# alexrenz/AdaPM

Measured on AMD Instinct MI355X. Metric: pull_push_ops_per_s, higher is better.
Workload: dtype fp32; 1 GPU; model=kge_complex_dim512, entities=10000000, relations=1000, dim=512, neg_samples=16, global_batch=16384, triples=90000000, parallelism=ps-async-dp1, fused_step=True, warmup_extra_steps=400

## Files before the change

adapm_amd/csrc/core.cpp:

```cpp
#include <torch/extension.h>
#include <ATen/Parallel.h>

#include <algorithm>
#include <atomic>
#include <condition_variable>
#include <cstring>
#include <limits>
#include <deque>
#include <map>
#include <queue>
#include <tuple>
#include <memory>
#include <mutex>
#include <random>
#include <thread>
#include <chrono>
#include <unordered_map>
#include <unordered_set>
#include <cstdio>
#include <vector>

#include "common.h"
#include "kernels.h"
#include "ops.h"
// ... 229 lines not shown
    adopt(current_stream(dev_));
    state_.copy_(h);
  }

  std::vector<uint64_t> export_state() {
    torch::Tensor h;
    {
      std::lock_guard<std::mutex> g(mu_);
      adopt(current_stream(dev_));
      h = state_.slice(0, 0, USTREAM_GEN_WORDS).cpu();
    }
    const uint64_t* p = reinterpret_cast<const uint64_t*>(h.data_ptr<int64_t>());
    return std::vector<uint64_t>(p, p + USTREAM_GEN_WORDS);
  }

  torch::Tensor draw(int64_t n, int64_t slack = -1) {
    TORCH_CHECK(n >= 0, "UniformStream.draw: n must be >= 0");
    auto opt = torch::TensorOptions().dtype(torch::kInt64).device(dev_);
    auto out = torch::empty({n}, opt);
    if (n == 0) return out;
    if (slack < 0) {
      double p = (double)thr_ / 4294967296.0;
      double w0 = (double)n / (1.0 - p);
      slack = (int64_t)std::ceil(w0 - (double)n + 8.0 * std::sqrt(w0 * p) / (1.0 - p)) + 16;
    }
    const int64_t words = n + slack;
    std::lock_guard<std::mutex> g(mu_);
    void* st = current_stream(dev_);
    adopt(st);
    auto tmp = torch::empty({ustream_tmp_words(words)}, opt);
    uint64_t* sp = reinterpret_cast<uint64_t*>(state_.data_ptr<int64_t>());
    if (dev_.is_cuda()) {
#ifdef ADAPM_WITH_HIP
      uniform_draw_gpu(sp, lo_, excl_, thr_, n, words, out.data_ptr<int64_t>(),
                       tmp.data_ptr<int64_t>(), st);
#else
      TORCH_CHECK(false, "UniformStream: built without HIP");
#endif
    } else {
      uniform_draw_cpu(sp, lo_, excl_, thr_, n, words, out.data_ptr<int64_t>(),
                       tmp.data_ptr<int64_t>());
    }
    return out;
  }

  int64_t lo() const { return lo_; }
  int64_t hi() const { return hi_; }
  const torch::Device& device() const { return dev_; }

 private:
// ... 2223 lines not shown
      const int64_t n = t->numel();
      for (int64_t i = 0; i < n; ++i) {
        int64_t k = kp[i];
        dst[i] = k;
        bad |= ((uint64_t)k >= lim);
      }
      dst += n;
    }
    if (bad)
      for (auto* t : parts) check_key_range(*t);
    hk.blob = blob;
    return hk;
  }

  StagedKeys upload_keys(const char* name, const HostKeys& hk, uint32_t* tags = nullptr,
                         const int64_t* dev_keys = nullptr, int64_t n_dev = 0) {
    const torch::Tensor& blob = hk.blob;
    const int64_t total = blob.numel();
    StagedKeys sk;
    sk.dev = torch::empty({total}, torch::TensorOptions().dtype(torch::kInt64).device(dev_));
#ifdef ADAPM_WITH_HIP
    auto stream = c10::hip::getCurrentHIPStreamMasqueradingAsCUDA(dev_.index());
    const bool ok =
        tags ? keys_land_gpu(tags, sk.dev.data_ptr<int64_t>(), blob.data_ptr<int64_t>(), total,
                             dev_keys, n_dev, (void*)stream.stream())
             : copy_keys_gpu(sk.dev.data_ptr<int64_t>(), blob.data_ptr<int64_t>(), total,
                             (void*)stream.stream());
    TORCH_CHECK(ok, name, ": the pinned key staging buffer is not visible to the device");
    at::getHostAllocator(at::kCUDA)->record_event(
        blob.data_ptr(), blob.storage().data_ptr().get_context(), stream.unwrap());
#else
    TORCH_CHECK(false, name, ": built without HIP");
#endif
    const int64_t* dp = sk.dev.data_ptr<int64_t>();
    for (int64_t n : hk.n) {
      sk.ptr.push_back(dp);
      dp += n;
    }
    return sk;
  }

  std::tuple<torch::Tensor, torch::Tensor> kge_step_fused_impl(
      const torch::Tensor& keys_s, const torch::Tensor& keys_r, const torch::Tensor& keys_o,
// ... 4 lines not shown
    int64_t B = keys_s.numel();
    TORCH_CHECK(keys_r.numel() == B && keys_o.numel() == B);
    TORCH_CHECK(N >= 0 && (3 + N) * B < (int64_t)ROWTAG_SHARED,
                "kge_step_fused: too many keys in one step");
    HostKeys hk;
    StagedKeys sk;
    torch::Tensor drawn;
    const int64_t* kn = nullptr;
    if (us) {
      TORCH_CHECK(us->lo() >= 0 && us->hi() <= num_keys_, "kge_step_fused_sampled: stream range [",
                  us->lo(), ", ", us->hi(), ") exceeds the store's ", num_keys_, " keys");
      TORCH_CHECK(us->device() == dev_,
                  "kge_step_fused_sampled: stream is not on the store's device");
      TORCH_CHECK(N >= 0 && B * N > 0, "kge_step_fused_sampled: nothing to draw");
      hk = host_keys({&keys_s, &keys_r, &keys_o});
      drawn = us->draw(B * N);
      kn = drawn.data_ptr<int64_t>();
    } else {
      TORCH_CHECK(keys_neg->numel() == B * N);
      hk = host_keys({&keys_s, &keys_r, &keys_o, keys_neg});
    }
    const int64_t n_dev = us ? B * N : 0;

    auto loss = torch::empty({B}, torch::TensorOptions().dtype(torch::kFloat32).device(dev_));
    void* st = current_stream(dev_);
    {
      InflightGuard g(this);
      std::unique_lock<std::mutex> mg(fused_mu_);
      if (fused_plain_ok(st)) {
        auto* tags = reinterpret_cast<uint32_t*>(fused_tags_.data_ptr<int32_t>());
        uint32_t* bits = tags + 32 * rowtag_words(num_keys_);
        sk = upload_keys("kge_step_fused", hk, tags, kn, n_dev);
        if (!us) kn = sk.ptr[3];
        RowTagKeys tk{{sk.ptr[0], kn, nullptr, nullptr}, {hk.blob.numel(), n_dev, 0, 0}, 2};
        rowtag_flag_gpu(tags, tk, st);
        rowtag_bits_gpu(tags, bits, tk, st);
        kge_complex_step_fused_gpu(
            slab_.data, sk.ptr[0], sk.ptr[1], sk.ptr[2], kn, loss.data_ptr<float>(), (int)B,
            (int)N, (int)D, Slab::padded(uniform_len_), world_, (float)lr, (float)eps, st, bits,
            fused_shared_stat_.defined()
                ? reinterpret_cast<unsigned long long*>(fused_shared_stat_.data_ptr<int64_t>())
                : nullptr);
        stat_fused_plain_ += 1;
      } else {
        mg.unlock();
        sk = upload_keys("kge_step_fused", hk);
        if (!us) kn = sk.ptr[3];
        kge_complex_step_fused_gpu(slab_.data, sk.ptr[0], sk.ptr[1], sk.ptr[2], kn,
                                   loss.data_ptr<float>(), (int)B, (int)N, (int)D,
                                   Slab::padded(uniform_len_), world_, (float)lr, (float)eps, st);
        stat_fused_atomic_ += 1;
      }
    }
    count_fused_ops(3 * B + B * N);
    return {loss, drawn};
  }

  torch::Tensor kge_step_fused(torch::Tensor keys_s, torch::Tensor keys_r, torch::Tensor keys_o,
                               torch::Tensor keys_neg, int64_t N, int64_t D, double lr,
                               double eps) {
// ... 44 lines not shown
    const int64_t n_dev = us ? B * (N + NS) : 0;

    auto loss = torch::empty({B}, torch::TensorOptions().dtype(torch::kFloat32).device(dev_));
    void* st = current_stream(dev_);
    {
      InflightGuard g(this);
      std::unique_lock<std::mutex> mg(fused_mu_);
      const bool plain = fused_plain_ok(st);
      uint32_t *tags = nullptr, *bits = nullptr;
      if (plain) {
        tags = reinterpret_cast<uint32_t*>(fused_tags_.data_ptr<int32_t>());
        bits = tags + 32 * rowtag_words(num_keys_);
      } else {
        mg.unlock();
      }
      sk = upload_keys(name, hk, tags, kno, n_dev);
      if (!us) kno = sk.ptr[3], kns = sk.ptr[4];
      if (plain) {
        RowTagKeys tk{{sk.ptr[0], kno, nullptr, nullptr}, {hk.blob.numel(), n_dev, 0, 0}, 2};
        rowtag_flag_gpu(tags, tk, st);
        rowtag_bits_gpu(tags, bits, tk, st);
      }
      kge_complex_step_sides_fused_gpu(
          slab_.data, sk.ptr[0], sk.ptr[1], sk.ptr[2], kno, kns, loss.data_ptr<float>(), (int)B,
          (int)N, (int)NS, (int)D, Slab::padded(uniform_len_), world_, (float)lr, (float)eps,
          (float)gamma_e, (float)gamma_r, st, bits,
          plain && fused_shared_stat_.defined()
              ? reinterpret_cast<unsigned long long*>(fused_shared_stat_.data_ptr<int64_t>())
              : nullptr);
      (plain ? stat_fused_plain_ : stat_fused_atomic_) += 1;
    }
    count_fused_ops(3 * B + B * (N + NS));
    return {loss, drawn};
  }

  torch::Tensor kge_step_sides_fused(torch::Tensor keys_s, torch::Tensor keys_r,
                                     torch::Tensor keys_o, torch::Tensor keys_neg_o,
                                     torch::Tensor keys_neg_s, int64_t N, int64_t NS, int64_t D,
                                     double lr, double eps, double gamma_e, double gamma_r) {
    return std::get<0>(kge_step_sides_fused_impl(keys_s, keys_r, keys_o, &keys_neg_o,
                                                 &keys_neg_s, nullptr, N, NS, D, lr, eps,
                                                 gamma_e, gamma_r));
  }

// ... 1126 lines not shown
    total += n;
  }
  TORCH_CHECK(total < (int64_t)ROWTAG_SHARED, "rowtag_shared_mask: too many occurrences");
  const int64_t words = rowtag_words(num_keys);
  auto tags = torch::empty({33 * words}, torch::TensorOptions().dtype(torch::kInt32).device(dev));
  auto* tp = reinterpret_cast<uint32_t*>(tags.data_ptr<int32_t>());
  void* st = current_stream(dev);
  rowtag_tag_gpu(tp, tk, st);
  rowtag_flag_gpu(tp, tk, st);
  rowtag_bits_gpu(tp, tp + 32 * words, tk, st);
  auto all = torch::cat(dk);
  auto word = tags.narrow(0, 32 * words, words).index_select(0, all.div(32, "floor"));
  return word.bitwise_right_shift(all.remainder(32).to(torch::kInt32)).bitwise_and(1).eq(1);
}

}

PYBIND11_MODULE(TORCH_EXTENSION_NAME, m) {
  using namespace adapm;
  m.def("hip_available", &hip_available);
  m.def("kge_complex_step", &kge_complex_step, py::call_guard<py::gil_scoped_release>());
  m.def("kge_complex_step_sides", &kge_complex_step_sides,
        py::call_guard<py::gil_scoped_release>());
  m.def("alias_draw", &alias_draw, py::call_guard<py::gil_scoped_release>());
  m.def("rescal_step", &rescal_step, py::call_guard<py::gil_scoped_release>());
  m.def("rescal_step_grouped", &rescal_step_grouped, py::call_guard<py::gil_scoped_release>());
  m.def("kge_complex_score", &kge_complex_score, py::call_guard<py::gil_scoped_release>());
  m.def("rank_count", &rank_count, py::arg("q"), py::arg("cand"), py::arg("base"),
        py::arg("counts"), py::arg("K"), py::arg("max_blocks") = 0,
        py::call_guard<py::gil_scoped_release>());
  m.def("pair_scores", &pair_scores, py::arg("q"), py::arg("cand"), py::arg("owner"),
        py::arg("out"), py::arg("K"), py::call_guard<py::gil_scoped_release>());
  m.def("w2v_sgns_step", &w2v_sgns_step, py::call_guard<py::gil_scoped_release>());
  m.def("mf_update_step", &mf_update_step, py::call_guard<py::gil_scoped_release>());
  m.def("mf_loss", &mf_loss, py::call_guard<py::gil_scoped_release>());
  m.def("slab_op", &slab_op, py::arg("op"), py::arg("dev"), py::arg("host"), py::arg("src_off"),
        py::arg("dst_off"), py::arg("lens"), py::arg("aux_off"), py::arg("buf"), py::arg("set"),
        py::call_guard<py::gil_scoped_release>());
  m.def("slab_keys_op", &slab_keys_op, py::arg("op"), py::arg("dev"), py::arg("keys"),
        py::arg("len"), py::arg("plen"), py::arg("world"), py::arg("rank"), py::arg("buf"),
        py::arg("set"), py::call_guard<py::gil_scoped_release>());
  m.def("rowtag_shared_mask", &rowtag_shared_mask, py::arg("keys"), py::arg("num_keys"),
        py::call_guard<py::gil_scoped_release>());
  py::class_<UniformStream>(m, "UniformStream")
      .def(py::init<int64_t, int64_t, std::string>(), py::arg("lo"), py::arg("hi"),
           py::arg("device"))
      .def_static("supported", &UniformStream::supported)
      .def("import_state", &UniformStream::import_state, py::call_guard<py::gil_scoped_release>())
      .def("export_state", &UniformStream::export_state, py::call_guard<py::gil_scoped_release>())
      .def("draw", &UniformStream::draw, py::arg("n"), py::arg("slack") = -1,
           py::call_guard<py::gil_scoped_release>())
      .def("lo", &UniformStream::lo)
      .def("hi", &UniformStream::hi);
  py::class_<Server>(m, "Server")
      .def(py::init<int64_t, torch::Tensor, int, int, int, int, std::string, double, int, bool,
                    int64_t, int64_t, double>(),
           py::arg("num_keys"), py::arg("value_lengths"), py::arg("rank"), py::arg("world"),
           py::arg("num_channels"), py::arg("num_workers"), py::arg("device"),
           py::arg("capacity_factor") = 2.0, py::arg("techniques") = 0,
           py::arg("location_caches") = true, py::arg("device_cap_floats") = 0,
           py::arg("host_spill_floats") = 0, py::arg("sync_threshold") = 0.0)
      .def("pull", &Server::pull, py::call_guard<py::gil_scoped_release>())
      .def("push", &Server::push, py::call_guard<py::gil_scoped_release>())
      .def("pull_if_local", &Server::pull_if_local, py::call_guard<py::gil_scoped_release>())
      .def("is_local", &Server::is_local)
      .def("intent", &Server::intent, py::call_guard<py::gil_scoped_release>())
      .def("advance_clock", &Server::advance_clock)
      .def("current_clock", &Server::current_clock)
// ... 57 lines not shown
```

adapm_amd/csrc/kernels.h:

```cpp
#pragma once
#include <cstdint>

namespace adapm {

constexpr int STEP_MAX_LANES = 8 * 256;

void kge_complex_step_gpu(const float* s, const float* r, const float* o, const float* neg,
                          float* ds, float* dr, float* do_, float* dneg, float* loss,
                          int B, int N, int D, float lr, float eps, void* stream);
void kge_complex_step_cpu(const float* s, const float* r, const float* o, const float* neg,
                          float* ds, float* dr, float* do_, float* dneg, float* loss,
                          int B, int N, int D, float lr, float eps);

void kge_complex_step_sides_gpu(const float* s, const float* r, const float* o,
                                const float* neg_o, const float* neg_s, float* ds, float* dr,
                                float* do_, float* dneg_o, float* dneg_s, float* loss, int B,
                                int N, int NS, int D, float lr, float eps, float gamma_e,
                                float gamma_r, void* stream);
void kge_complex_step_sides_cpu(const float* s, const float* r, const float* o,
                                const float* neg_o, const float* neg_s, float* ds, float* dr,
                                float* do_, float* dneg_o, float* dneg_s, float* loss, int B,
                                int N, int NS, int D, float lr, float eps, float gamma_e,
                                float gamma_r);

constexpr uint32_t ROWTAG_SHARED = 0xFFFFFFFFu;
struct RowTagKeys {
  const int64_t* keys[4];
  int64_t n[4];
  int count;
};
inline int64_t rowtag_words(int64_t rows) { return (rows + 31) / 32; }
void rowtag_tag_gpu(uint32_t* tags, const RowTagKeys& ks, void* stream);
void rowtag_flag_gpu(uint32_t* tags, const RowTagKeys& ks, void* stream);
void rowtag_bits_gpu(const uint32_t* tags, uint32_t* bits, const RowTagKeys& ks, void* stream);

bool keys_land_gpu(uint32_t* tags, int64_t* dst, const int64_t* src_host, int64_t n_copy,
                   const int64_t* dev_keys, int64_t n_dev, void* stream);

void kge_complex_step_fused_gpu(float* slab, const int64_t* keys_s, const int64_t* keys_r,
                                const int64_t* keys_o, const int64_t* keys_neg, float* loss,
                                int B, int N, int D, int32_t plen, int world, float lr,
                                float eps, void* stream, const uint32_t* bits = nullptr,
                                unsigned long long* shared_stat = nullptr);

void kge_complex_step_sides_fused_gpu(float* slab, const int64_t* keys_s, const int64_t* keys_r,
                                      const int64_t* keys_o, const int64_t* keys_neg_o,
                                      const int64_t* keys_neg_s, float* loss, int B, int N,
                                      int NS, int D, int32_t plen, int world, float lr,
                                      float eps, float gamma_e, float gamma_r, void* stream,
                                      const uint32_t* bits = nullptr,
                                      unsigned long long* shared_stat = nullptr);
void kge_complex_step_sides_fused_offs_cpu(float* slab, const int64_t* offs_s,
                                           const int64_t* offs_r, const int64_t* offs_o,
                                           const int64_t* offs_neg_o, const int64_t* offs_neg_s,
                                           float* loss, int B, int N, int NS, int D, float lr,
                                           float eps, float gamma_e, float gamma_r);

void kge_complex_step_fused_offs_cpu(float* slab, const int64_t* offs_s, const int64_t* offs_r,
                                     const int64_t* offs_o, const int64_t* offs_neg, float* loss,
                                     int B, int N, int D, float lr, float eps);
void w2v_sgns_step_fused_offs_cpu(float* slab, const int64_t* offs_ctr, const int64_t* offs_ctx,
                                  const int64_t* offs_neg, float* loss, int B, int N, int D,
                                  float lr, float eps);
void mf_update_step_fused_offs_cpu(float* slab, const int64_t* offs_w, const int64_t* offs_h,
                                   const float* x, float* loss, int B, int R, float lr,
                                   float lambda, float eps);
// ... 29 lines not shown
                        float* loss, int B, int R, float lr, float lambda, float eps,
                        void* stream);
void mf_update_step_cpu(const float* w, const float* h, const float* x, float* dw, float* dh,
                        float* loss, int B, int R, float lr, float lambda, float eps);

void mf_loss_gpu(const float* w, const float* h, const float* x, double* acc2, int B, int R,
                 float lambda, void* stream);
void mf_loss_cpu(const float* w, const float* h, const float* x, float* out2, int B, int R,
                 float lambda);

void alias_draw_gpu(const float* prob, const int32_t* alias, int64_t n, uint64_t seed,
                    int64_t N, int64_t* out, void* stream);
void alias_draw_cpu(const float* prob, const int32_t* alias, int64_t n, uint64_t seed,
                    int64_t N, int64_t* out);

void uniform_draw_gpu(uint64_t* state, int64_t lo, uint32_t excl, uint32_t thr, int64_t n,
                      int64_t words, int64_t* out, int64_t* tmp, void* stream);
void uniform_draw_cpu(uint64_t* state, int64_t lo, uint32_t excl, uint32_t thr, int64_t n,
                      int64_t words, int64_t* out, int64_t* tmp);

bool copy_keys_gpu(int64_t* dst, const int64_t* src_host, int64_t n, void* stream);

}

namespace adapm {


void kge_complex_score_mfma_gpu(const float* s, const float* r, const float* cand,
                                float* scores, float* qbuf, int B, int E, int D, void* stream);

void rank_count_gpu(const float* Q, const float* C, const float* base, int32_t* counts, int B,
                    int E, int K, int qstride, int cstride, int max_blocks, void* stream);
// ... 22 lines not shown
```

adapm_amd/csrc/kernels_hip.hip:

```cpp
#include <hip/hip_runtime.h>
#include <algorithm>
#include <type_traits>

#include "kernels.h"
#include "ustream.h"

namespace adapm {

#define KT 256

static inline unsigned grid_for(int64_t n, int64_t cap = 16384) {
  return (unsigned)std::min(std::max<int64_t>(n, 1), cap);
}

static_assert(STEP_MAX_LANES == 8 * KT, "dispatch_kpt stops at KPT = 8");
template <typename F>
static inline void dispatch_kpt(int lanes, F&& f) {
  if (lanes <= KT) f(std::integral_constant<int, 1>{});
  else if (lanes <= 2 * KT) f(std::integral_constant<int, 2>{});
  else if (lanes <= 4 * KT) f(std::integral_constant<int, 4>{});
  else f(std::integral_constant<int, 8>{});
}

__device__ inline float block_reduce_sum(float v, float* lds) {
// ... 462 lines not shown
}

namespace adapm {
void alias_draw_gpu(const float* prob, const int32_t* alias, int64_t n, uint64_t seed,
                    int64_t N, int64_t* out, void* stream) {
  if (N == 0) return;
  hipLaunchKernelGGL(k_alias_draw, dim3(grid_for((N + 255) / 256, 4096)), dim3(256), 0,
                     (hipStream_t)stream, prob, alias, n, seed, N, out);
}
}

namespace adapm {

static_assert(USTREAM_BLOCK == KT, "one chunk per thread of a KT workgroup");

__device__ inline int64_t block_reduce_i64(int64_t v, int64_t* lds) {
  for (int off = 32; off > 0; off >>= 1) v += __shfl_xor(v, off, 64);
  if ((threadIdx.x & 63) == 0) lds[threadIdx.x >> 6] = v;
  __syncthreads();
  int64_t out = 0;
  for (int i = 0; i < KT / 64; ++i) out += lds[i];
  __syncthreads();
  return out;
}

template <typename T>
__device__ inline T* ustream_block_keys(T* tmp, int64_t nb, int64_t block) {
  return tmp + USTREAM_TMP_COUNTS + nb + block * (KT * USTREAM_CHUNK) + threadIdx.x;
}

__global__ void __launch_bounds__(KT)
k_ustream_gen(const uint64_t* __restrict__ state, UStreamRange r, int64_t words, int64_t chunks,
              int64_t* __restrict__ tmp, int64_t nb) {
  __shared__ int64_t lds[KT / 64];
  const int64_t c = (int64_t)blockIdx.x * KT + threadIdx.x;
  int64_t cnt = 0;
  if (c < chunks)
    cnt = ustream_gen_chunk(state, r, words, c, ustream_block_keys(tmp, nb, blockIdx.x), KT);
  cnt = block_reduce_i64(cnt, lds);
  if (threadIdx.x == 0) {
    tmp[USTREAM_TMP_COUNTS + blockIdx.x] = cnt;
  }
}

__global__ void __launch_bounds__(KT)
k_ustream_compact(uint64_t* __restrict__ state, UStreamRange r, int64_t n, int64_t words,
                  int64_t chunks, const int64_t* __restrict__ tmp, int64_t nb,
                  int64_t* __restrict__ out) {
  __shared__ int64_t lds[KT / 64];
  __shared__ int wave_tot[KT / 64];
  const int64_t* counts = tmp + USTREAM_TMP_COUNTS;
  int64_t part = 0;
  for (int64_t i = threadIdx.x; i < (int64_t)blockIdx.x; i += KT) part += counts[i];
  const int64_t off = block_reduce_i64(part, lds);
  const int64_t c = (int64_t)blockIdx.x * KT + threadIdx.x;
  const bool live = off < n && c < chunks;
  const int64_t* kc = ustream_block_keys(tmp, nb, blockIdx.x);
  int64_t k[USTREAM_CHUNK];
  int cnt = 0;
#pragma unroll
  for (int i = 0; i < USTREAM_CHUNK; ++i) {
    k[i] = live ? kc[i * KT] : USTREAM_REJECTED;
    cnt += (k[i] != USTREAM_REJECTED);
// ... 2 lines not shown
  int incl = cnt;
  for (int d = 1; d < 64; d <<= 1) {
    int y = __shfl_up(incl, d, 64);
    if (lane >= d) incl += y;
  }
  if (lane == 63) wave_tot[wave] = incl;
  __syncthreads();
  int64_t idx = off + incl - cnt;
  for (int i = 0; i < wave; ++i) idx += wave_tot[i];
  int64_t consumed = 0;
#pragma unroll
  for (int i = 0; i < USTREAM_CHUNK; ++i) {
    if (k[i] == USTREAM_REJECTED) continue;
    if (idx < n) {
      out[idx] = k[i];
      if (idx == n - 1) consumed = c * USTREAM_CHUNK + i + 1;
    }
    ++idx;
  }
  if (consumed) {
    ustream_finish(state, r, n, words, n, consumed, out);
  } else if (blockIdx.x == nb - 1 && threadIdx.x == 0) {
    int64_t total = off;
    for (int i = 0; i < KT / 64; ++i) total += wave_tot[i];
    if (total < n) ustream_finish(state, r, n, words, total, 0, out);
  }
}

void uniform_draw_gpu(uint64_t* state, int64_t lo, uint32_t excl, uint32_t thr, int64_t n,
                      int64_t words, int64_t* out, int64_t* tmp, void* stream) {
  if (n <= 0) return;
  const UStreamRange r{lo, excl, thr};
  const int64_t chunks = ustream_chunks(words), nb = ustream_blocks(words);
  auto st = (hipStream_t)stream;
  hipLaunchKernelGGL(k_ustream_gen, dim3((unsigned)nb), dim3(KT), 0, st, state, r, words, chunks,
                     tmp, nb);
  hipLaunchKernelGGL(k_ustream_compact, dim3((unsigned)nb), dim3(KT), 0, st, state, r, n, words,
                     chunks, tmp, nb, out);
}

__global__ void k_copy_keys(int64_t* __restrict__ dst, const int64_t* __restrict__ src,
                            int64_t n) {
  int64_t i = (int64_t)blockIdx.x * KT + threadIdx.x;
  if (i < n) dst[i] = src[i];
}

bool copy_keys_gpu(int64_t* dst, const int64_t* src_host, int64_t n, void* stream) {
  if (n <= 0) return true;
  void* src = nullptr;
  if (hipHostGetDevicePointer(&src, const_cast<int64_t*>(src_host), 0) != hipSuccess || !src) {
    (void)hipGetLastError();
    return false;
  }
// ... 96 lines not shown
    ++a;
  }
  return ks.keys[a][i];
}

__device__ inline void rowtag_tag(uint32_t* tags, int64_t row, int64_t i) {
  tags[row] = (uint32_t)i;
}

__device__ inline void rowtag_flag(uint32_t* tags, int64_t row, int64_t i) {
  if (tags[row] != (uint32_t)i) tags[row] = ROWTAG_SHARED;
}

__global__ void k_keys_land(uint32_t* __restrict__ tags, int64_t* __restrict__ dst,
                            const int64_t* __restrict__ src, int64_t n_copy,
                            const int64_t* __restrict__ dev_keys, int64_t total) {
  int64_t i = (int64_t)blockIdx.x * KT + threadIdx.x;
  if (i >= total) return;
  int64_t row;
  if (i < n_copy) {
    row = src[i];
    dst[i] = row;
  } else {
    row = dev_keys[i - n_copy];
  }
  rowtag_tag(tags, row, i);
}

__global__ void k_rowtag_tag(uint32_t* __restrict__ tags, RowTagKeys ks, int64_t total) {
  int64_t i = (int64_t)blockIdx.x * KT + threadIdx.x;
  if (i >= total) return;
  rowtag_tag(tags, rowtag_key(ks, i), i);
}

__global__ void k_rowtag_flag(uint32_t* __restrict__ tags, RowTagKeys ks, int64_t total) {
  int64_t i = (int64_t)blockIdx.x * KT + threadIdx.x;
  if (i >= total) return;
  rowtag_flag(tags, rowtag_key(ks, i), i);
}

__global__ void k_rowtag_bits(const uint32_t* __restrict__ tags, uint32_t* __restrict__ bits,
// ... 1 lines not shown
  int64_t i = (int64_t)blockIdx.x * KT + threadIdx.x;
  if (i >= total) return;
  const int64_t w = rowtag_key(ks, i) >> 5;
  const uint4* t = reinterpret_cast<const uint4*>(tags + (w << 5));
  uint32_t word = 0;
#pragma unroll
  for (int q = 0; q < 8; ++q) {
    const uint4 v = t[q];
    word |= ((uint32_t)(v.x == ROWTAG_SHARED) | (uint32_t)(v.y == ROWTAG_SHARED) << 1 |
             (uint32_t)(v.z == ROWTAG_SHARED) << 2 | (uint32_t)(v.w == ROWTAG_SHARED) << 3)
            << (4 * q);
  }
  bits[w] = word;
}

static int64_t rowtag_total(const RowTagKeys& ks) {
  int64_t total = 0;
  for (int a = 0; a < ks.count; ++a) total += ks.n[a];
  return total;
}

void rowtag_tag_gpu(uint32_t* tags, const RowTagKeys& ks, void* stream) {
  const int64_t total = rowtag_total(ks);
  if (total == 0) return;
  hipLaunchKernelGGL(k_rowtag_tag, dim3((unsigned)((total + KT - 1) / KT)), dim3(KT), 0,
                     (hipStream_t)stream, tags, ks, total);
}

void rowtag_flag_gpu(uint32_t* tags, const RowTagKeys& ks, void* stream) {
  const int64_t total = rowtag_total(ks);
  if (total == 0) return;
  hipLaunchKernelGGL(k_rowtag_flag, dim3((unsigned)((total + KT - 1) / KT)), dim3(KT), 0,
                     (hipStream_t)stream, tags, ks, total);
}

void rowtag_bits_gpu(const uint32_t* tags, uint32_t* bits, const RowTagKeys& ks, void* stream) {
  const int64_t total = rowtag_total(ks);
  if (total == 0) return;
  hipLaunchKernelGGL(k_rowtag_bits, dim3((unsigned)((total + KT - 1) / KT)), dim3(KT), 0,
                     (hipStream_t)stream, tags, bits, ks, total);
}

bool keys_land_gpu(uint32_t* tags, int64_t* dst, const int64_t* src_host, int64_t n_copy,
                   const int64_t* dev_keys, int64_t n_dev, void* stream) {
  const int64_t total = n_copy + n_dev;
  if (total <= 0) return true;
  void* src = nullptr;
  if (n_copy > 0 &&
      (hipHostGetDevicePointer(&src, const_cast<int64_t*>(src_host), 0) != hipSuccess || !src)) {
    (void)hipGetLastError();
    return false;
  }
  hipLaunchKernelGGL(k_keys_land, dim3((unsigned)((total + KT - 1) / KT)), dim3(KT), 0,
                     (hipStream_t)stream, tags, dst, static_cast<const int64_t*>(src), n_copy,
                     dev_keys, total);
  return true;
}

template <bool UNIQ>
__device__ inline bool row_shared(const uint32_t* __restrict__ bits, int64_t key) {
  if (!UNIQ) return true;
  return (bits[key >> 5] >> (int)(key & 31)) & 1u;
}

__device__ inline float plain_add(float a, float delta) {
#pragma clang fp contract(off)
  return a + delta;
}

__device__ inline void slab_adagrad(float* p_emb, float* p_acc, float g, float emb, float acc,
// ... 15 lines not shown
    float d_re = -lr * (g_re) * __frsqrt_rn(G_re + eps);                              \
    float d_im = -lr * (g_im) * __frsqrt_rn(G_im + eps);                              \
    if (shared) {                                                                     \
      atomicAdd(&(row)[k], d_re);                                                     \
      atomicAdd(&(row)[dc + k], d_im);                                                \
      atomicAdd(&(row)[D + k], (g_re) * (g_re));                                      \
      atomicAdd(&(row)[D + dc + k], (g_im) * (g_im));                                 \
    } else {                                                                          \
      (row)[k] = plain_add(emb_re, d_re);                                             \
      (row)[dc + k] = plain_add(emb_im, d_im);                                        \
      (row)[D + k] = plain_add(acc_re, (g_re) * (g_re));                              \
      (row)[D + dc + k] = plain_add(acc_im, (g_im) * (g_im));                         \
    }                                                                                 \
  } while (0)

template <int KPT, bool UNIQ>
__global__ void k_kge_step_fused(float* __restrict__ slab, const int64_t* __restrict__ keys_s,
                                 const int64_t* __restrict__ keys_r,
                                 const int64_t* __restrict__ keys_o,
                                 const int64_t* __restrict__ keys_neg, float* __restrict__ loss,
                                 int B, int N, int D, int32_t plen, int world, float lr,
                                 float eps, const uint32_t* __restrict__ bits,
                                 unsigned long long* __restrict__ shared_stat) {
  __shared__ float lds[KT / 64];
  const int dc = D >> 1;
  const int w = UNIQ ? 1 : world;
  for (int b = blockIdx.x; b < B; b += gridDim.x) {
    const int64_t key_s = keys_s[b], key_r = keys_r[b];
    const float* sb = row_at(slab, key_s, plen, w);
    const float* rb = row_at(slab, key_r, plen, w);
    const bool s_shared = row_shared<UNIQ>(bits, key_s);
    const bool r_shared = row_shared<UNIQ>(bits, key_r);
    unsigned n_shared = (unsigned)s_shared + (unsigned)r_shared;

    float s_re[KPT], s_im[KPT], r_re[KPT], r_im[KPT];
    float a_sre[KPT], a_sim[KPT], a_rre[KPT], a_rim[KPT];
    float u_re[KPT], u_im[KPT];
#pragma unroll
    for (int i = 0; i < KPT; ++i) {
      int k = threadIdx.x + i * KT;
      a_sre[i] = a_sim[i] = a_rre[i] = a_rim[i] = 0.f;
      if (k < dc) {
        s_re[i] = sb[k];
        s_im[i] = sb[dc + k];
        r_re[i] = rb[k];
        r_im[i] = rb[dc + k];
        u_re[i] = s_re[i] * r_re[i] - s_im[i] * r_im[i];
        u_im[i] = s_im[i] * r_re[i] + s_re[i] * r_im[i];
      } else {
        s_re[i] = s_im[i] = r_re[i] = r_im[i] = u_re[i] = u_im[i] = 0.f;
      }
    }

    float lsum = 0.f;
    for (int j = 0; j <= N; ++j) {
      int64_t ok = (j == 0) ? keys_o[b] : keys_neg[(int64_t)b * N + (j - 1)];
      float* ob = row_at(slab, ok, plen, w);
      const bool o_shared = row_shared<UNIQ>(bits, ok);
      n_shared += (unsigned)o_shared;
      float y = (j == 0) ? 1.f : -1.f;
      float part = 0.f;
      float o_re[KPT], o_im[KPT], Go_re[KPT], Go_im[KPT];
#pragma unroll
      for (int i = 0; i < KPT; ++i) {
        int k = threadIdx.x + i * KT;
        o_re[i] = k < dc ? ob[k] : 0.f;
        o_im[i] = k < dc ? ob[dc + k] : 0.f;
        Go_re[i] = k < dc ? ob[D + k] : 0.f;
        Go_im[i] = k < dc ? ob[D + dc + k] : 0.f;
        part += u_re[i] * o_re[i] + u_im[i] * o_im[i];
      }
      float psi = block_reduce_sum(part, lds);
      float c = -y * sigmoidf(-y * psi);
// ... 2 lines not shown
#pragma unroll
      for (int i = 0; i < KPT; ++i) {
        int k = threadIdx.x + i * KT;
        if (k >= dc) continue;
        a_sre[i] += c * (r_re[i] * o_re[i] + r_im[i] * o_im[i]);
        a_sim[i] += c * (r_re[i] * o_im[i] - r_im[i] * o_re[i]);
        a_rre[i] += c * (s_re[i] * o_re[i] + s_im[i] * o_im[i]);
        a_rim[i] += c * (s_re[i] * o_im[i] - s_im[i] * o_re[i]);
        float g_re = c * u_re[i];
        float g_im = c * u_im[i];
        SLAB_ADAGRAD_COMPLEX(ob, o_shared, g_re, g_im, o_re[i], o_im[i], Go_re[i], Go_im[i]);
      }
    }
    float* dsb = const_cast<float*>(sb);
    float* drb = const_cast<float*>(rb);
#pragma unroll
    for (int i = 0; i < KPT; ++i) {
      int k = threadIdx.x + i * KT;
      if (k >= dc) continue;
      float Gs_re = sb[D + k], Gs_im = sb[D + dc + k];
      SLAB_ADAGRAD_COMPLEX(dsb, s_shared, a_sre[i], a_sim[i], s_re[i], s_im[i], Gs_re, Gs_im);
      float Gr_re = rb[D + k], Gr_im = rb[D + dc + k];
      SLAB_ADAGRAD_COMPLEX(drb, r_shared, a_rre[i], a_rim[i], r_re[i], r_im[i], Gr_re, Gr_im);
    }
    if (threadIdx.x == 0) {
      loss[b] = lsum;
      if (UNIQ && shared_stat) atomicAdd(shared_stat, (unsigned long long)n_shared);
    }
  }
}

#undef SLAB_ADAGRAD_COMPLEX

void kge_complex_step_fused_gpu(float* slab, const int64_t* keys_s, const int64_t* keys_r,
                                const int64_t* keys_o, const int64_t* keys_neg, float* loss,
                                int B, int N, int D, int32_t plen, int world, float lr,
                                float eps, void* stream, const uint32_t* bits,
                                unsigned long long* shared_stat) {
  if (B < 1) return;
  const bool uniq = bits != nullptr && world == 1;
  if (!uniq) bits = nullptr, shared_stat = nullptr;
  dispatch_kpt(D >> 1, [&](auto kpt) {
    constexpr int KPT = decltype(kpt)::value;
    hipLaunchKernelGGL((uniq ? k_kge_step_fused<KPT, true> : k_kge_step_fused<KPT, false>),
                       dim3(grid_for(B)), dim3(KT), 0, (hipStream_t)stream, slab, keys_s, keys_r,
                       keys_o, keys_neg, loss, B, N, D, plen, world, lr, eps, bits,
                       shared_stat);
  });
}

__device__ inline void slab_adagrad_complex(float* row, int k, int dc, int D, float g_re,
                                            float g_im, float emb_re, float emb_im, float acc_re,
                                            float acc_im, float lr, float eps, bool shared) {
  slab_adagrad(&row[k], &row[D + k], g_re, emb_re, acc_re, lr, eps, shared);
  slab_adagrad(&row[dc + k], &row[D + dc + k], g_im, emb_im, acc_im, lr, eps, shared);
}

template <int KPT, bool UNIQ>
__global__ void __launch_bounds__(KT)
k_kge_step_sides_fused(float* __restrict__ slab, const int64_t* __restrict__ keys_s,
                       const int64_t* __restrict__ keys_r, const int64_t* __restrict__ keys_o,
// ... 139 lines not shown
                           a_oim[i] + gamma_e * p_im[i], p_re[i], p_im[i], pb[D + k],
                           pb[D + dc + k], lr, eps, p_shared);
    }
    if (threadIdx.x == 0) {
      loss[b] = lsum;
      if (UNIQ && shared_stat) atomicAdd(shared_stat, (unsigned long long)n_shared);
    }
  }
}

void kge_complex_step_sides_fused_gpu(float* slab, const int64_t* keys_s, const int64_t* keys_r,
                                      const int64_t* keys_o, const int64_t* keys_neg_o,
                                      const int64_t* keys_neg_s, float* loss, int B, int N,
                                      int NS, int D, int32_t plen, int world, float lr,
                                      float eps, float gamma_e, float gamma_r, void* stream,
                                      const uint32_t* bits, unsigned long long* shared_stat) {
  if (B < 1) return;
  if (NS == 0 && gamma_e == 0.f && gamma_r == 0.f)
    return kge_complex_step_fused_gpu(slab, keys_s, keys_r, keys_o, keys_neg_o, loss, B, N, D,
                                      plen, world, lr, eps, stream, bits, shared_stat);
  const bool uniq = bits != nullptr && world == 1;
  if (!uniq) bits = nullptr, shared_stat = nullptr;
  dispatch_kpt(D >> 1, [&](auto kpt) {
    constexpr int KPT = decltype(kpt)::value;
    hipLaunchKernelGGL(
        (uniq ? k_kge_step_sides_fused<KPT, true> : k_kge_step_sides_fused<KPT, false>),
        dim3(grid_for(B)), dim3(KT), 0, (hipStream_t)stream, slab, keys_s, keys_r, keys_o,
        keys_neg_o, keys_neg_s, loss, B, N, NS, D, plen, world, lr, eps, gamma_e, gamma_r, bits,
        shared_stat);
  });
}

}

namespace adapm {
// ... 95 lines not shown
```

Measured before the change: 1.302 billion key-ops/s.

## Track shared rows per occurrence and fuse key landing into uniform draw

Replaces the per-row shared bitmap (tag pass, flag pass, bits pass over num_keys words) with a per-occurrence byte array. The kernel reads it through a wavefront ballot instead of random bitmap lookups. Host-key landing and tagging are folded into extra blocks of the uniform-stream generation kernel, so the separate keys_land launch goes away, and the bits-building kernel over the whole key space is dropped. The cost is an extra per-step device allocation for the occurrence array. The flag pass can also write to other occurrences' bytes, which is benign.

Result: slower. 1.059 billion key-ops/s (-18.7%).

```diff
diff --git a/adapm_amd/csrc/core.cpp b/adapm_amd/csrc/core.cpp
--- a/adapm_amd/csrc/core.cpp
+++ b/adapm_amd/csrc/core.cpp
@@ -267,8 +267,12 @@
     return std::vector<uint64_t>(p, p + USTREAM_GEN_WORDS);
   }
 
-  torch::Tensor draw(int64_t n, int64_t slack = -1) {
+  torch::Tensor draw(int64_t n, int64_t slack = -1) { return draw_land(n, slack, nullptr); }
+
+  torch::Tensor draw_land(int64_t n, int64_t slack, const KeysLandOcc* land) {
     TORCH_CHECK(n >= 0, "UniformStream.draw: n must be >= 0");
+    TORCH_CHECK(!land || (n > 0 && dev_.is_cuda() && lo_ >= 0),
+                "UniformStream.draw: a landing request needs a GPU stream of row keys and n > 0");
     auto opt = torch::TensorOptions().dtype(torch::kInt64).device(dev_);
     auto out = torch::empty({n}, opt);
     if (n == 0) return out;
@@ -285,8 +289,10 @@
     uint64_t* sp = reinterpret_cast<uint64_t*>(state_.data_ptr<int64_t>());
     if (dev_.is_cuda()) {
 #ifdef ADAPM_WITH_HIP
-      uniform_draw_gpu(sp, lo_, excl_, thr_, n, words, out.data_ptr<int64_t>(),
-                       tmp.data_ptr<int64_t>(), st);
+      const bool ok = uniform_draw_gpu(sp, lo_, excl_, thr_, n, words, out.data_ptr<int64_t>(),
+                                       tmp.data_ptr<int64_t>(), st, land);
+      TORCH_CHECK(ok, "UniformStream.draw: the pinned key staging buffer is not visible to "
+                      "the device");
 #else
       TORCH_CHECK(false, "UniformStream: built without HIP");
 #endif
@@ -2540,19 +2546,27 @@
   }
 
   StagedKeys upload_keys(const char* name, const HostKeys& hk, uint32_t* tags = nullptr,
-                         const int64_t* dev_keys = nullptr, int64_t n_dev = 0) {
+                         const int64_t* dev_keys = nullptr, int64_t n_dev = 0,
+                         uint8_t* occ = nullptr, UniformStream* us = nullptr,
+                         torch::Tensor* drawn = nullptr) {
     const torch::Tensor& blob = hk.blob;
     const int64_t total = blob.numel();
     StagedKeys sk;
     sk.dev = torch::empty({total}, torch::TensorOptions().dtype(torch::kInt64).device(dev_));
 #ifdef ADAPM_WITH_HIP
     auto stream = c10::hip::getCurrentHIPStreamMasqueradingAsCUDA(dev_.index());
-    const bool ok =
-        tags ? keys_land_gpu(tags, sk.dev.data_ptr<int64_t>(), blob.data_ptr<int64_t>(), total,
-                             dev_keys, n_dev, (void*)stream.stream())
-             : copy_keys_gpu(sk.dev.data_ptr<int64_t>(), blob.data_ptr<int64_t>(), total,
-                             (void*)stream.stream());
-    TORCH_CHECK(ok, name, ": the pinned key staging buffer is not visible to the device");
+    if (us) {
+      const KeysLandOcc land{tags, occ, sk.dev.data_ptr<int64_t>(), blob.data_ptr<int64_t>(),
+                             total};
+      *drawn = us->draw_land(n_dev, -1, &land);
+    } else {
+      const bool ok =
+          tags ? keys_land_gpu(tags, sk.dev.data_ptr<int64_t>(), blob.data_ptr<int64_t>(), total,
+                               dev_keys, n_dev, (void*)stream.stream(), occ)
+               : copy_keys_gpu(sk.dev.data_ptr<int64_t>(), blob.data_ptr<int64_t>(), total,
+                               (void*)stream.stream());
+      TORCH_CHECK(ok, name, ": the pinned key staging buffer is not visible to the device");
+    }
     at::getHostAllocator(at::kCUDA)->record_event(
         blob.data_ptr(), blob.storage().data_ptr().get_context(), stream.unwrap());
 #else
@@ -2587,8 +2601,6 @@
                   "kge_step_fused_sampled: stream is not on the store's device");
       TORCH_CHECK(N >= 0 && B * N > 0, "kge_step_fused_sampled: nothing to draw");
       hk = host_keys({&keys_s, &keys_r, &keys_o});
-      drawn = us->draw(B * N);
-      kn = drawn.data_ptr<int64_t>();
     } else {
       TORCH_CHECK(keys_neg->numel() == B * N);
       hk = host_keys({&keys_s, &keys_r, &keys_o, keys_neg});
@@ -2602,21 +2614,26 @@
       std::unique_lock<std::mutex> mg(fused_mu_);
       if (fused_plain_ok(st)) {
         auto* tags = reinterpret_cast<uint32_t*>(fused_tags_.data_ptr<int32_t>());
-        uint32_t* bits = tags + 32 * rowtag_words(num_keys_);
-        sk = upload_keys("kge_step_fused", hk, tags, kn, n_dev);
-        if (!us) kn = sk.ptr[3];
+        auto occ_t = torch::empty({(3 + N) * B},
+                                  torch::TensorOptions().dtype(torch::kUInt8).device(dev_));
+        uint8_t* occ = occ_t.data_ptr<uint8_t>();
+        sk = upload_keys("kge_step_fused", hk, tags, nullptr, n_dev, occ, us, &drawn);
+        kn = us ? drawn.data_ptr<int64_t>() : sk.ptr[3];
         RowTagKeys tk{{sk.ptr[0], kn, nullptr, nullptr}, {hk.blob.numel(), n_dev, 0, 0}, 2};
-        rowtag_flag_gpu(tags, tk, st);
-        rowtag_bits_gpu(tags, bits, tk, st);
+        rowocc_flag_gpu(tags, occ, tk, st);
         kge_complex_step_fused_gpu(
             slab_.data, sk.ptr[0], sk.ptr[1], sk.ptr[2], kn, loss.data_ptr<float>(), (int)B,
-            (int)N, (int)D, Slab::padded(uniform_len_), world_, (float)lr, (float)eps, st, bits,
+            (int)N, (int)D, Slab::padded(uniform_len_), world_, (float)lr, (float)eps, st, occ,
             fused_shared_stat_.defined()
                 ? reinterpret_cast<unsigned long long*>(fused_shared_stat_.data_ptr<int64_t>())
                 : nullptr);
         stat_fused_plain_ += 1;
       } else {
         mg.unlock();
+        if (us) {
+          drawn = us->draw(B * N);
+          kn = drawn.data_ptr<int64_t>();
+        }
         sk = upload_keys("kge_step_fused", hk);
         if (!us) kn = sk.ptr[3];
         kge_complex_step_fused_gpu(slab_.data, sk.ptr[0], sk.ptr[1], sk.ptr[2], kn,
@@ -2691,12 +2708,24 @@
       } else {
         mg.unlock();
       }
-      sk = upload_keys(name, hk, tags, kno, n_dev);
+      const bool one_sided = kge_sides_is_one_sided((int)NS, (float)gamma_e, (float)gamma_r);
+      torch::Tensor occ_t;
+      uint8_t* occ = nullptr;
+      if (plain && one_sided) {
+        occ_t = torch::empty({(3 + N + NS) * B},
+                             torch::TensorOptions().dtype(torch::kUInt8).device(dev_));
+        occ = occ_t.data_ptr<uint8_t>();
+      }
+      sk = upload_keys(name, hk, tags, kno, n_dev, occ);
       if (!us) kno = sk.ptr[3], kns = sk.ptr[4];
       if (plain) {
         RowTagKeys tk{{sk.ptr[0], kno, nullptr, nullptr}, {hk.blob.numel(), n_dev, 0, 0}, 2};
-        rowtag_flag_gpu(tags, tk, st);
-        rowtag_bits_gpu(tags, bits, tk, st);
+        if (one_sided) {
+          rowocc_flag_gpu(tags, occ, tk, st);
+        } else {
+          rowtag_flag_gpu(tags, tk, st);
+          rowtag_bits_gpu(tags, bits, tk, st);
+        }
       }
       kge_complex_step_sides_fused_gpu(
           slab_.data, sk.ptr[0], sk.ptr[1], sk.ptr[2], kno, kns, loss.data_ptr<float>(), (int)B,
@@ -2704,7 +2733,8 @@
           (float)gamma_e, (float)gamma_r, st, bits,
           plain && fused_shared_stat_.defined()
               ? reinterpret_cast<unsigned long long*>(fused_shared_stat_.data_ptr<int64_t>())
-              : nullptr);
+              : nullptr,
+          occ);
       (plain ? stat_fused_plain_ : stat_fused_atomic_) += 1;
     }
     count_fused_ops(3 * B + B * (N + NS));
@@ -3861,6 +3891,75 @@
   return word.bitwise_right_shift(all.remainder(32).to(torch::kInt32)).bitwise_and(1).eq(1);
 }
 
+torch::Tensor rowtag_shared_occ(std::vector<torch::Tensor> keys, int64_t num_keys) {
+  TORCH_CHECK(hip_available(), "rowtag_shared_occ: no HIP device");
+  TORCH_CHECK(!keys.empty() && keys.size() <= 4, "rowtag_shared_occ: one to four key arrays");
+  TORCH_CHECK(num_keys >= 1 && num_keys <= std::numeric_limits<int32_t>::max(),
+              "rowtag_shared_occ: bad num_keys");
+  const torch::Device dev(torch::kCUDA, c10::hip::current_device());
+  std::vector<torch::Tensor> dk;
+  RowTagKeys tk{{nullptr, nullptr, nullptr, nullptr}, {0, 0, 0, 0}, (int)keys.size()};
+  int64_t total = 0;
+  for (size_t a = 0; a < keys.size(); ++a) {
+    const int64_t n = keys[a].numel();
+    check_host_batch_tensor(keys[a], torch::kInt64, n, "keys");
+    const int64_t* kp = keys[a].data_ptr<int64_t>();
+    for (int64_t i = 0; i < n; ++i)
+      TORCH_CHECK(kp[i] >= 0 && kp[i] < num_keys, "rowtag_shared_occ: key out of range: ", kp[i]);
+    dk.push_back(keys[a].to(dev));
+    tk.keys[a] = dk.back().data_ptr<int64_t>();
+    tk.n[a] = n;
+    total += n;
+  }
+  TORCH_CHECK(total < (int64_t)ROWTAG_SHARED, "rowtag_shared_occ: too many occurrences");
+  auto tags = torch::empty({num_keys}, torch::TensorOptions().dtype(torch::kInt32).device(dev));
+  auto occ = torch::empty({total}, torch::TensorOptions().dtype(torch::kUInt8).device(dev));
+  auto* tp = reinterpret_cast<uint32_t*>(tags.data_ptr<int32_t>());
+  void* st = current_stream(dev);
+  rowocc_tag_gpu(tp, occ.data_ptr<uint8_t>(), tk, st);
+  rowocc_flag_gpu(tp, occ.data_ptr<uint8_t>(), tk, st);
+  return occ.eq(1);
+}
+
+std::tuple<torch::Tensor, torch::Tensor> uniform_draw_land(UniformStream& us, int64_t n,
+                                                           int64_t slack,
+                                                           torch::Tensor host_keys,
+                                                           int64_t num_keys) {
+  TORCH_CHECK(hip_available(), "uniform_draw_land: no HIP device");
+  TORCH_CHECK(num_keys >= 1 && num_keys <= std::numeric_limits<int32_t>::max(),
+              "uniform_draw_land: bad num_keys");
+  TORCH_CHECK(n > 0, "uniform_draw_land: nothing to draw");
+  TORCH_CHECK(us.device().is_cuda() && us.lo() >= 0 && us.hi() <= num_keys,
+              "uniform_draw_land: needs a GPU stream whose range lies within num_keys");
+  const int64_t h = host_keys.numel();
+  check_host_batch_tensor(host_keys, torch::kInt64, h, "host_keys");
+  TORCH_CHECK(h + n < (int64_t)ROWTAG_SHARED, "uniform_draw_land: too many occurrences");
+  const torch::Device dev = us.device();
+  auto blob = torch::empty({h}, torch::TensorOptions().dtype(torch::kInt64).pinned_memory(true));
+  const int64_t* kp = host_keys.data_ptr<int64_t>();
+  for (int64_t i = 0; i < h; ++i) {
+    TORCH_CHECK(kp[i] >= 0 && kp[i] < num_keys, "uniform_draw_land: key out of range: ", kp[i]);
+    blob.data_ptr<int64_t>()[i] = kp[i];
+  }
+  auto tags = torch::empty({num_keys}, torch::TensorOptions().dtype(torch::kInt32).device(dev));
+  auto occ = torch::empty({h + n}, torch::TensorOptions().dtype(torch::kUInt8).device(dev));
+  auto landed = torch::empty({h}, torch::TensorOptions().dtype(torch::kInt64).device(dev));
+  auto* tp = reinterpret_cast<uint32_t*>(tags.data_ptr<int32_t>());
+  const KeysLandOcc land{tp, occ.data_ptr<uint8_t>(), landed.data_ptr<int64_t>(),
+                         blob.data_ptr<int64_t>(), h};
+  torch::Tensor drawn = us.draw_land(n, slack, &land);
+  if (h > 0) {
+    auto stream = c10::hip::getCurrentHIPStreamMasqueradingAsCUDA(dev.index());
+    at::getHostAllocator(at::kCUDA)->record_event(
+        blob.data_ptr(), blob.storage().data_ptr().get_context(), stream.unwrap());
+  }
+  RowTagKeys tk{{landed.data_ptr<int64_t>(), drawn.data_ptr<int64_t>(), nullptr, nullptr},
+                {h, n, 0, 0},
+                2};
+  rowocc_flag_gpu(tp, occ.data_ptr<uint8_t>(), tk, current_stream(dev));
+  return {drawn, occ.eq(1)};
+}
+
 }
 
 PYBIND11_MODULE(TORCH_EXTENSION_NAME, m) {
@@ -3889,6 +3988,8 @@
         py::arg("set"), py::call_guard<py::gil_scoped_release>());
   m.def("rowtag_shared_mask", &rowtag_shared_mask, py::arg("keys"), py::arg("num_keys"),
         py::call_guard<py::gil_scoped_release>());
+  m.def("rowtag_shared_occ", &rowtag_shared_occ, py::arg("keys"), py::arg("num_keys"),
+        py::call_guard<py::gil_scoped_release>());
   py::class_<UniformStream>(m, "UniformStream")
       .def(py::init<int64_t, int64_t, std::string>(), py::arg("lo"), py::arg("hi"),
            py::arg("device"))
@@ -3899,6 +4000,9 @@
            py::call_guard<py::gil_scoped_release>())
       .def("lo", &UniformStream::lo)
       .def("hi", &UniformStream::hi);
+  m.def("uniform_draw_land", &uniform_draw_land, py::arg("stream"), py::arg("n"),
+        py::arg("slack"), py::arg("host_keys"), py::arg("num_keys"),
+        py::call_guard<py::gil_scoped_release>());
   py::class_<Server>(m, "Server")
       .def(py::init<int64_t, torch::Tensor, int, int, int, int, std::string, double, int, bool,
                     int64_t, int64_t, double>(),
diff --git a/adapm_amd/csrc/kernels.h b/adapm_amd/csrc/kernels.h
--- a/adapm_amd/csrc/kernels.h
+++ b/adapm_amd/csrc/kernels.h
@@ -35,21 +35,37 @@
 void rowtag_bits_gpu(const uint32_t* tags, uint32_t* bits, const RowTagKeys& ks, void* stream);
 
 bool keys_land_gpu(uint32_t* tags, int64_t* dst, const int64_t* src_host, int64_t n_copy,
-                   const int64_t* dev_keys, int64_t n_dev, void* stream);
+                   const int64_t* dev_keys, int64_t n_dev, void* stream,
+                   uint8_t* occ = nullptr);
+
+void rowocc_tag_gpu(uint32_t* tags, uint8_t* occ, const RowTagKeys& ks, void* stream);
+void rowocc_flag_gpu(const uint32_t* tags, uint8_t* occ, const RowTagKeys& ks, void* stream);
+
+struct KeysLandOcc {
+  uint32_t* tags;
+  uint8_t* occ;
+  int64_t* dst;
+  const int64_t* src;
+  int64_t n;
+};
 
 void kge_complex_step_fused_gpu(float* slab, const int64_t* keys_s, const int64_t* keys_r,
                                 const int64_t* keys_o, const int64_t* keys_neg, float* loss,
                                 int B, int N, int D, int32_t plen, int world, float lr,
-                                float eps, void* stream, const uint32_t* bits = nullptr,
+                                float eps, void* stream, const uint8_t* occ = nullptr,
                                 unsigned long long* shared_stat = nullptr);
 
+inline bool kge_sides_is_one_sided(int NS, float gamma_e, float gamma_r) {
+  return NS == 0 && gamma_e == 0.f && gamma_r == 0.f;
+}
 void kge_complex_step_sides_fused_gpu(float* slab, const int64_t* keys_s, const int64_t* keys_r,
                                       const int64_t* keys_o, const int64_t* keys_neg_o,
                                       const int64_t* keys_neg_s, float* loss, int B, int N,
                                       int NS, int D, int32_t plen, int world, float lr,
                                       float eps, float gamma_e, float gamma_r, void* stream,
                                       const uint32_t* bits = nullptr,
-                                      unsigned long long* shared_stat = nullptr);
+                                      unsigned long long* shared_stat = nullptr,
+                                      const uint8_t* occ = nullptr);
 void kge_complex_step_sides_fused_offs_cpu(float* slab, const int64_t* offs_s,
                                            const int64_t* offs_r, const int64_t* offs_o,
                                            const int64_t* offs_neg_o, const int64_t* offs_neg_s,
@@ -109,8 +125,9 @@
 void alias_draw_cpu(const float* prob, const int32_t* alias, int64_t n, uint64_t seed,
                     int64_t N, int64_t* out);
 
-void uniform_draw_gpu(uint64_t* state, int64_t lo, uint32_t excl, uint32_t thr, int64_t n,
-                      int64_t words, int64_t* out, int64_t* tmp, void* stream);
+bool uniform_draw_gpu(uint64_t* state, int64_t lo, uint32_t excl, uint32_t thr, int64_t n,
+                      int64_t words, int64_t* out, int64_t* tmp, void* stream,
+                      const KeysLandOcc* land = nullptr);
 void uniform_draw_cpu(uint64_t* state, int64_t lo, uint32_t excl, uint32_t thr, int64_t n,
                       int64_t words, int64_t* out, int64_t* tmp);
 
diff --git a/adapm_amd/csrc/kernels_hip.hip b/adapm_amd/csrc/kernels_hip.hip
--- a/adapm_amd/csrc/kernels_hip.hip
+++ b/adapm_amd/csrc/kernels_hip.hip
@@ -500,6 +500,19 @@
 
 static_assert(USTREAM_BLOCK == KT, "one chunk per thread of a KT workgroup");
 
+__device__ inline void rowocc_tag(uint32_t* tags, uint8_t* occ, int64_t row, int64_t i) {
+  tags[row] = (uint32_t)i;
+  occ[i] = 0;
+}
+
+__device__ inline void rowocc_flag(const uint32_t* tags, uint8_t* occ, int64_t row, int64_t i) {
+  const uint32_t t = tags[row];
+  if (t != (uint32_t)i) {
+    occ[i] = 1;
+    occ[t] = 1;
+  }
+}
+
 __device__ inline int64_t block_reduce_i64(int64_t v, int64_t* lds) {
   for (int off = 32; off > 0; off >>= 1) v += __shfl_xor(v, off, 64);
   if ((threadIdx.x & 63) == 0) lds[threadIdx.x >> 6] = v;
@@ -517,8 +530,17 @@
 
 __global__ void __launch_bounds__(KT)
 k_ustream_gen(const uint64_t* __restrict__ state, UStreamRange r, int64_t words, int64_t chunks,
-              int64_t* __restrict__ tmp, int64_t nb) {
+              int64_t* __restrict__ tmp, int64_t nb, KeysLandOcc land) {
   __shared__ int64_t lds[KT / 64];
+  if ((int64_t)blockIdx.x >= nb) {
+    const int64_t i = ((int64_t)blockIdx.x - nb) * KT + threadIdx.x;
+    if (i < land.n) {
+      const int64_t row = land.src[i];
+      land.dst[i] = row;
+      rowocc_tag(land.tags, land.occ, row, i);
+    }
+    return;
+  }
   const int64_t c = (int64_t)blockIdx.x * KT + threadIdx.x;
   int64_t cnt = 0;
   if (c < chunks)
@@ -532,7 +554,7 @@
 __global__ void __launch_bounds__(KT)
 k_ustream_compact(uint64_t* __restrict__ state, UStreamRange r, int64_t n, int64_t words,
                   int64_t chunks, const int64_t* __restrict__ tmp, int64_t nb,
-                  int64_t* __restrict__ out) {
+                  int64_t* __restrict__ out, KeysLandOcc land) {
   __shared__ int64_t lds[KT / 64];
   __shared__ int wave_tot[KT / 64];
   const int64_t* counts = tmp + USTREAM_TMP_COUNTS;
@@ -565,6 +587,7 @@
     if (k[i] == USTREAM_REJECTED) continue;
     if (idx < n) {
       out[idx] = k[i];
+      if (land.tags) rowocc_tag(land.tags, land.occ, k[i], land.n + idx);
       if (idx == n - 1) consumed = c * USTREAM_CHUNK + i + 1;
     }
     ++idx;
@@ -574,20 +597,38 @@
   } else if (blockIdx.x == nb - 1 && threadIdx.x == 0) {
     int64_t total = off;
     for (int i = 0; i < KT / 64; ++i) total += wave_tot[i];
-    if (total < n) ustream_finish(state, r, n, words, total, 0, out);
-  }
-}
-
-void uniform_draw_gpu(uint64_t* state, int64_t lo, uint32_t excl, uint32_t thr, int64_t n,
-                      int64_t words, int64_t* out, int64_t* tmp, void* stream) {
-  if (n <= 0) return;
+    if (total < n) {
+      ustream_finish(state, r, n, words, total, 0, out);
+      if (land.tags)
+        for (int64_t i = total; i < n; ++i) rowocc_tag(land.tags, land.occ, out[i], land.n + i);
+    }
+  }
+}
+
+bool uniform_draw_gpu(uint64_t* state, int64_t lo, uint32_t excl, uint32_t thr, int64_t n,
+                      int64_t words, int64_t* out, int64_t* tmp, void* stream,
+                      const KeysLandOcc* land) {
+  if (n <= 0) return true;
   const UStreamRange r{lo, excl, thr};
   const int64_t chunks = ustream_chunks(words), nb = ustream_blocks(words);
   auto st = (hipStream_t)stream;
-  hipLaunchKernelGGL(k_ustream_gen, dim3((unsigned)nb), dim3(KT), 0, st, state, r, words, chunks,
-                     tmp, nb);
+  KeysLandOcc l{nullptr, nullptr, nullptr, nullptr, 0};
+  if (land) {
+    l = *land;
+    void* src = nullptr;
+    if (l.n > 0 &&
+        (hipHostGetDevicePointer(&src, const_cast<int64_t*>(l.src), 0) != hipSuccess || !src)) {
+      (void)hipGetLastError();
+      return false;
+    }
+    l.src = static_cast<const int64_t*>(src);
+  }
+  const int64_t nb_land = (l.n + KT - 1) / KT;
+  hipLaunchKernelGGL(k_ustream_gen, dim3((unsigned)(nb + nb_land)), dim3(KT), 0, st, state, r,
+                     words, chunks, tmp, nb, l);
   hipLaunchKernelGGL(k_ustream_compact, dim3((unsigned)nb), dim3(KT), 0, st, state, r, n, words,
-                     chunks, tmp, nb, out);
+                     chunks, tmp, nb, out, l);
+  return true;
 }
 
 __global__ void k_copy_keys(int64_t* __restrict__ dst, const int64_t* __restrict__ src,
@@ -714,7 +755,8 @@
 
 __global__ void k_keys_land(uint32_t* __restrict__ tags, int64_t* __restrict__ dst,
                             const int64_t* __restrict__ src, int64_t n_copy,
-                            const int64_t* __restrict__ dev_keys, int64_t total) {
+                            const int64_t* __restrict__ dev_keys, int64_t total,
+                            uint8_t* __restrict__ occ) {
   int64_t i = (int64_t)blockIdx.x * KT + threadIdx.x;
   if (i >= total) return;
   int64_t row;
@@ -725,6 +767,7 @@
     row = dev_keys[i - n_copy];
   }
   rowtag_tag(tags, row, i);
+  if (occ) occ[i] = 0;
 }
 
 __global__ void k_rowtag_tag(uint32_t* __restrict__ tags, RowTagKeys ks, int64_t total) {
@@ -756,6 +799,20 @@
   bits[w] = word;
 }
 
+__global__ void k_rowocc_tag(uint32_t* __restrict__ tags, uint8_t* __restrict__ occ,
+                             RowTagKeys ks, int64_t total) {
+  int64_t i = (int64_t)blockIdx.x * KT + threadIdx.x;
+  if (i >= total) return;
+  rowocc_tag(tags, occ, rowtag_key(ks, i), i);
+}
+
+__global__ void k_rowocc_flag(const uint32_t* __restrict__ tags, uint8_t* __restrict__ occ,
+                              RowTagKeys ks, int64_t total) {
+  int64_t i = (int64_t)blockIdx.x * KT + threadIdx.x;
+  if (i >= total) return;
+  rowocc_flag(tags, occ, rowtag_key(ks, i), i);
+}
+
 static int64_t rowtag_total(const RowTagKeys& ks) {
   int64_t total = 0;
   for (int a = 0; a < ks.count; ++a) total += ks.n[a];
@@ -783,8 +840,22 @@
                      (hipStream_t)stream, tags, bits, ks, total);
 }
 
+void rowocc_tag_gpu(uint32_t* tags, uint8_t* occ, const RowTagKeys& ks, void* stream) {
+  const int64_t total = rowtag_total(ks);
+  if (total == 0) return;
+  hipLaunchKernelGGL(k_rowocc_tag, dim3((unsigned)((total + KT - 1) / KT)), dim3(KT), 0,
+                     (hipStream_t)stream, tags, occ, ks, total);
+}
+
+void rowocc_flag_gpu(const uint32_t* tags, uint8_t* occ, const RowTagKeys& ks, void* stream) {
+  const int64_t total = rowtag_total(ks);
+  if (total == 0) return;
+  hipLaunchKernelGGL(k_rowocc_flag, dim3((unsigned)((total + KT - 1) / KT)), dim3(KT), 0,
+                     (hipStream_t)stream, tags, occ, ks, total);
+}
+
 bool keys_land_gpu(uint32_t* tags, int64_t* dst, const int64_t* src_host, int64_t n_copy,
-                   const int64_t* dev_keys, int64_t n_dev, void* stream) {
+                   const int64_t* dev_keys, int64_t n_dev, void* stream, uint8_t* occ) {
   const int64_t total = n_copy + n_dev;
   if (total <= 0) return true;
   void* src = nullptr;
@@ -795,7 +866,7 @@
   }
   hipLaunchKernelGGL(k_keys_land, dim3((unsigned)((total + KT - 1) / KT)), dim3(KT), 0,
                      (hipStream_t)stream, tags, dst, static_cast<const int64_t*>(src), n_copy,
-                     dev_keys, total);
+                     dev_keys, total, occ);
   return true;
 }
 
@@ -841,13 +912,27 @@
     }                                                                                 \
   } while (0)
 
+
+__device__ inline uint64_t occ_mask(const uint8_t* __restrict__ occ, int B, int N, int b,
+                                    int i0) {
+  const int it = i0 + (int)(threadIdx.x & 63);
+  const int64_t at = it < 3 ? (int64_t)it * B + b : 3 * (int64_t)B + (int64_t)b * N + (it - 3);
+  return __ballot(it < N + 3 && occ[at] != 0);
+}
+
+template <bool UNIQ>
+__device__ inline bool occ_shared(uint64_t mask, int i) {
+  if (!UNIQ) return true;
+  return (mask >> (i & 63)) & 1;
+}
+
 template <int KPT, bool UNIQ>
 __global__ void k_kge_step_fused(float* __restrict__ slab, const int64_t* __restrict__ keys_s,
                                  const int64_t* __restrict__ keys_r,
                                  const int64_t* __restrict__ keys_o,
                                  const int64_t* __restrict__ keys_neg, float* __restrict__ loss,
                                  int B, int N, int D, int32_t plen, int world, float lr,
-                                 float eps, const uint32_t* __restrict__ bits,
+                                 float eps, const uint8_t* __restrict__ occ,
                                  unsigned long long* __restrict__ shared_stat) {
   __shared__ float lds[KT / 64];
   const int dc = D >> 1;
@@ -856,9 +941,9 @@
     const int64_t key_s = keys_s[b], key_r = keys_r[b];
     const float* sb = row_at(slab, key_s, plen, w);
     const float* rb = row_at(slab, key_r, plen, w);
-    const bool s_shared = row_shared<UNIQ>(bits, key_s);
-    const bool r_shared = row_shared<UNIQ>(bits, key_r);
-    unsigned n_shared = (unsigned)s_shared + (unsigned)r_shared;
+    uint64_t m_occ = UNIQ ? occ_mask(occ, B, N, b, 0) : 0;
+    const uint64_t m_sr = m_occ;
+    unsigned n_shared = 0;
 
     float s_re[KPT], s_im[KPT], r_re[KPT], r_im[KPT];
     float a_sre[KPT], a_sim[KPT], a_rre[KPT], a_rim[KPT];
@@ -883,7 +968,8 @@
     for (int j = 0; j <= N; ++j) {
       int64_t ok = (j == 0) ? keys_o[b] : keys_neg[(int64_t)b * N + (j - 1)];
       float* ob = row_at(slab, ok, plen, w);
-      const bool o_shared = row_shared<UNIQ>(bits, ok);
+      if (UNIQ && ((j + 2) & 63) == 0) m_occ = occ_mask(occ, B, N, b, j + 2);
+      const bool o_shared = occ_shared<UNIQ>(m_occ, j + 2);
       n_shared += (unsigned)o_shared;
       float y = (j == 0) ? 1.f : -1.f;
       float part = 0.f;
@@ -916,6 +1002,9 @@
     }
     float* dsb = const_cast<float*>(sb);
     float* drb = const_cast<float*>(rb);
+    const bool s_shared = occ_shared<UNIQ>(m_sr, 0);
+    const bool r_shared = occ_shared<UNIQ>(m_sr, 1);
+    n_shared += (unsigned)s_shared + (unsigned)r_shared;
 #pragma unroll
     for (int i = 0; i < KPT; ++i) {
       int k = threadIdx.x + i * KT;
@@ -937,16 +1026,16 @@
 void kge_complex_step_fused_gpu(float* slab, const int64_t* keys_s, const int64_t* keys_r,
                                 const int64_t* keys_o, const int64_t* keys_neg, float* loss,
                                 int B, int N, int D, int32_t plen, int world, float lr,
-                                float eps, void* stream, const uint32_t* bits,
+                                float eps, void* stream, const uint8_t* occ,
                                 unsigned long long* shared_stat) {
   if (B < 1) return;
-  const bool uniq = bits != nullptr && world == 1;
-  if (!uniq) bits = nullptr, shared_stat = nullptr;
+  const bool uniq = occ != nullptr && world == 1;
+  if (!uniq) occ = nullptr, shared_stat = nullptr;
   dispatch_kpt(D >> 1, [&](auto kpt) {
     constexpr int KPT = decltype(kpt)::value;
     hipLaunchKernelGGL((uniq ? k_kge_step_fused<KPT, true> : k_kge_step_fused<KPT, false>),
                        dim3(grid_for(B)), dim3(KT), 0, (hipStream_t)stream, slab, keys_s, keys_r,
-                       keys_o, keys_neg, loss, B, N, D, plen, world, lr, eps, bits,
+                       keys_o, keys_neg, loss, B, N, D, plen, world, lr, eps, occ,
                        shared_stat);
   });
 }
@@ -1116,11 +1205,12 @@
                                       const int64_t* keys_neg_s, float* loss, int B, int N,
                                       int NS, int D, int32_t plen, int world, float lr,
                                       float eps, float gamma_e, float gamma_r, void* stream,
-                                      const uint32_t* bits, unsigned long long* shared_stat) {
+                                      const uint32_t* bits, unsigned long long* shared_stat,
+                                      const uint8_t* occ) {
   if (B < 1) return;
-  if (NS == 0 && gamma_e == 0.f && gamma_r == 0.f)
+  if (kge_sides_is_one_sided(NS, gamma_e, gamma_r))
     return kge_complex_step_fused_gpu(slab, keys_s, keys_r, keys_o, keys_neg_o, loss, B, N, D,
-                                      plen, world, lr, eps, stream, bits, shared_stat);
+                                      plen, world, lr, eps, stream, occ, shared_stat);
   const bool uniq = bits != nullptr && world == 1;
   if (!uniq) bits = nullptr, shared_stat = nullptr;
   dispatch_kpt(D >> 1, [&](auto kpt) {
```
